# laclouis5/StructureDetector

Hardware: AMD Instinct MI355X
Metric: images/sec (train fwd+bwd) and decode us/img at 512x512 (higher is better)
Workload: dtype f32

## Files before the change

structuredetector_amd/csrc/sd_nn.hip:

```cpp
#include "sd_common.h"
#include "sd_mfma.h"
#include <type_traits>

namespace sd {

constexpr int RED_ROWS_PER_BLOCK = 256;

template <int MODE, typename T = float>
__global__ __launch_bounds__(256) void k_col_reduce(const T* __restrict__ a, const T* __restrict__ b, const T* __restrict__ y,
                                                     const float* __restrict__ mean, const float* __restrict__ invstd,
                                                     const float* __restrict__ gamma, const float* __restrict__ beta, int relu,
                                                     int64_t M, int C, float* __restrict__ partial, int rpb) {
    __shared__ float4 red[2][256];
    const int cols = C >> 2;
    const int lanes = 256 / cols;
    const int col = threadIdx.x % cols, rl = threadIdx.x / cols;
    const int64_t r0 = (int64_t)blockIdx.x * rpb;
    const int64_t r1 = min(r0 + rpb, M);
    float4 s0 = make_float4(0.f, 0.f, 0.f, 0.f), s1 = s0;
    float4 mu = s0, is = s0, ga = s0, be = s0;
    if (MODE == 1 && rl < lanes) {
        mu = reinterpret_cast<const float4*>(mean)[col];
        is = reinterpret_cast<const float4*>(invstd)[col];
        if (relu == 2) { ga = reinterpret_cast<const float4*>(gamma)[col]; be = reinterpret_cast<const float4*>(beta)[col]; }
    }
    if (rl < lanes) {
#pragma unroll 4
        for (int64_t r = r0 + rl; r < r1; r += lanes) {
            const float4 v = ld4(a, r * cols + col);
            if (MODE == 0) {
                s0.x += v.x; s0.y += v.y; s0.z += v.z; s0.w += v.w;
                s1.x += v.x * v.x; s1.y += v.y * v.y; s1.z += v.z * v.z; s1.w += v.w * v.w;
            } else if (MODE == 2) {
                s0.x += v.x; s0.y += v.y; s0.z += v.z; s0.w += v.w;
            } else {
                float4 g = v;
                const float4 xv = ld4(b, r * cols + col);
                if (relu == 1) {
                    const float4 yy = ld4(y, r * cols + col);
                    g.x = yy.x > 0.f ? g.x : 0.f; g.y = yy.y > 0.f ? g.y : 0.f;
                    g.z = yy.z > 0.f ? g.z : 0.f; g.w = yy.w > 0.f ? g.w : 0.f;
                } else if (relu == 2) {
                    g.x = ((xv.x - mu.x) * is.x * ga.x + be.x) > 0.f ? g.x : 0.f; g.y = ((xv.y - mu.y) * is.y * ga.y + be.y) > 0.f ? g.y : 0.f;
                    g.z = ((xv.z - mu.z) * is.z * ga.z + be.z) > 0.f ? g.z : 0.f; g.w = ((xv.w - mu.w) * is.w * ga.w + be.w) > 0.f ? g.w : 0.f;
                } else if (relu == 3) {
                    const uint8_t mb = reinterpret_cast<const uint8_t*>(y)[r * cols + col];
                    g.x = (mb & 1) ? g.x : 0.f; g.y = (mb & 2) ? g.y : 0.f; g.z = (mb & 4) ? g.z : 0.f; g.w = (mb & 8) ? g.w : 0.f;
                }
                s0.x += g.x; s0.y += g.y; s0.z += g.z; s0.w += g.w;
                s1.x += g.x * ((xv.x - mu.x) * is.x); s1.y += g.y * ((xv.y - mu.y) * is.y);
                s1.z += g.z * ((xv.z - mu.z) * is.z); s1.w += g.w * ((xv.w - mu.w) * is.w);
            }
        }
    }
    red[0][threadIdx.x] = s0;
    red[1][threadIdx.x] = s1;
    __syncthreads();
    if (rl == 0) {
        for (int l = 1; l < lanes; ++l) {
            const float4 u = red[0][l * cols + col], w = red[1][l * cols + col];
            s0.x += u.x; s0.y += u.y; s0.z += u.z; s0.w += u.w;
            s1.x += w.x; s1.y += w.y; s1.z += w.z; s1.w += w.w;
        }
        float* dst = partial + (int64_t)blockIdx.x * 2 * C;
        reinterpret_cast<float4*>(dst)[col] = s0;
        reinterpret_cast<float4*>(dst + C)[col] = s1;
    }
}

__global__ __launch_bounds__(256) void k_rows_fold(const float* __restrict__ in, int rows, int W, int slab, float* __restrict__ out) {
    __shared__ float4 red[256];
    const int cols = W >> 2, lanes = 256 / cols;
    const int col = threadIdx.x % cols, rl = threadIdx.x / cols;
    const int r0 = blockIdx.x * slab, r1 = min(r0 + slab, rows);
    float4 s = make_float4(0.f, 0.f, 0.f, 0.f);
    if (rl < lanes) {
#pragma unroll 4
        for (int r = r0 + rl; r < r1; r += lanes) {
            const float4 v = reinterpret_cast<const float4*>(in + (int64_t)r * W)[col];
            s.x += v.x; s.y += v.y; s.z += v.z; s.w += v.w;
        }
    }
    red[threadIdx.x] = s;
    __syncthreads();
    if (rl == 0) {
        for (int l = 1; l < lanes; ++l) { const float4 u = red[l * cols + col]; s.x += u.x; s.y += u.y; s.z += u.z; s.w += u.w; }
        reinterpret_cast<float4*>(out + (int64_t)blockIdx.x * W)[col] = s;
    }
}

__device__ __forceinline__ bool col_pair_sums(const float* __restrict__ partial, int nblocks, int C, double (&r0)[4][4], double (&r1)[4][4],
                                              double& s0, double& s1) {
    const int lc = threadIdx.x & 3, lr = threadIdx.x >> 2;
    const int c = blockIdx.x * 4 + lc;
    s0 = 0.0; s1 = 0.0;
    if (c < C) {
        double t0[8] = {0, 0, 0, 0, 0, 0, 0, 0}, t1[8] = {0, 0, 0, 0, 0, 0, 0, 0};
        for (int b = lr; b < nblocks; b += 64 * 8) {
            float v0[8], v1[8];
#pragma unroll
            for (int u = 0; u < 8; ++u) {
                const int row = b + 64 * u;
                const int64_t o = (int64_t)(row < nblocks ? row : 0) * 2 * C + c;
                v0[u] = partial[o];
                v1[u] = partial[o + C];
            }
#pragma unroll
            for (int u = 0; u < 8; ++u) {
                const bool ok = b + 64 * u < nblocks;
                t0[u] += ok ? (double)v0[u] : 0.0; t1[u] += ok ? (double)v1[u] : 0.0;
            }
        }
        s0 = ((t0[0] + t0[1]) + (t0[2] + t0[3])) + ((t0[4] + t0[5]) + (t0[6] + t0[7]));
        s1 = ((t1[0] + t1[1]) + (t1[2] + t1[3])) + ((t1[4] + t1[5]) + (t1[6] + t1[7]));
    }
#pragma unroll
    for (int o = 4; o < 64; o <<= 1) { s0 += __shfl_xor(s0, o); s1 += __shfl_xor(s1, o); }
// ... 26 lines not shown
    __shared__ double r0[4][4], r1[4][4];
    double s0, s1;
    if (!col_pair_sums(partial, nblocks, C, r0, r1, s0, s1)) return;
    const int c = blockIdx.x * 4 + (threadIdx.x & 3);
    if (FIN == 0) {
        bn_stats_tail(s0, s1, M, eps, momentum, c, out0, out1, run_mean, run_var);
    } else if (FIN == 1) {
        out0[c] = (accumulate ? out0[c] : 0.f) + (float)s1;
        out1[c] = (accumulate ? out1[c] : 0.f) + (float)s0;
        aux0[c] = (float)(s0 / M);
        aux1[c] = (float)(s1 / M);
    } else {
        out0[c] = (accumulate ? out0[c] : 0.f) + (float)s0;
    }
}

template <int FIN>
__global__ __launch_bounds__(256) void k_col_sums(const float* __restrict__ partial, int nblocks, int C, double M, float* __restrict__ dgamma,
                                                   float* __restrict__ dbeta, int accumulate, double* __restrict__ sums) {
    __shared__ double r0[4][4], r1[4][4];
    double s0, s1;
    if (!col_pair_sums(partial, nblocks, C, r0, r1, s0, s1)) return;
    const int c = blockIdx.x * 4 + (threadIdx.x & 3);
    sums[c] = s0;
    sums[C + c] = s1;
    if (c == 0) sums[2 * C] = M;
    if (FIN == 1) {
        dgamma[c] = (accumulate ? dgamma[c] : 0.f) + (float)s1;
        dbeta[c] = (accumulate ? dbeta[c] : 0.f) + (float)s0;
    }
}

__global__ __launch_bounds__(256) void k_bn_stats_from_sums(const double* __restrict__ sums, int C, float eps, float momentum,
                                                             float* __restrict__ mean, float* __restrict__ invstd,
                                                             float* __restrict__ run_mean, float* __restrict__ run_var) {
    const int c = blockIdx.x * 256 + threadIdx.x;
    if (c >= C) return;
    bn_stats_tail(sums[c], sums[C + c], sums[2 * C], eps, momentum, c, mean, invstd, run_mean, run_var);
}

__global__ __launch_bounds__(256) void k_bn_bwd_means_from_sums(const double* __restrict__ sums, int C, float* __restrict__ means) {
    const int c = blockIdx.x * 256 + threadIdx.x;
    if (c >= C) return;
    const double M = sums[2 * C];
    means[c] = (float)(sums[c] / M);
    means[C + c] = (float)(sums[C + c] / M);
}

template <typename T>
__global__ __launch_bounds__(256) void k_bn_apply(const T* __restrict__ x, T* __restrict__ y, int64_t n4, int C,
                                                   const float* __restrict__ mean, const float* __restrict__ invstd,
                                                   const float* __restrict__ gamma, const float* __restrict__ beta,
                                                   const T* __restrict__ res, int relu, uint8_t* __restrict__ mask) {
    const int64_t stride = (int64_t)gridDim.x * 256;
    const int cols = C >> 2;
    const bool fixed = stride % cols == 0;
    const int col0 = (int)(((int64_t)blockIdx.x * 256 + threadIdx.x) % cols);
    float4 mu = reinterpret_cast<const float4*>(mean)[col0], is = reinterpret_cast<const float4*>(invstd)[col0];
    float4 g = reinterpret_cast<const float4*>(gamma)[col0], b = reinterpret_cast<const float4*>(beta)[col0];
    for (int64_t i = (int64_t)blockIdx.x * 256 + threadIdx.x; i < n4; i += stride) {
        const float4 v = ld4(x, i);
        if (!fixed) {
            const int col = (int)(i % cols);
            mu = reinterpret_cast<const float4*>(mean)[col]; is = reinterpret_cast<const float4*>(invstd)[col];
            g = reinterpret_cast<const float4*>(gamma)[col]; b = reinterpret_cast<const float4*>(beta)[col];
        }
        float4 o;
        o.x = (v.x - mu.x) * is.x * g.x + b.x; o.y = (v.y - mu.y) * is.y * g.y + b.y;
        o.z = (v.z - mu.z) * is.z * g.z + b.z; o.w = (v.w - mu.w) * is.w * g.w + b.w;
        if (res) {
            const float4 r = ld4(res, i);
            o.x += r.x; o.y += r.y; o.z += r.z; o.w += r.w;
        }
        if (mask) mask[i] = (uint8_t)((o.x > 0.f ? 1 : 0) | (o.y > 0.f ? 2 : 0) | (o.z > 0.f ? 4 : 0) | (o.w > 0.f ? 8 : 0));
        if (relu) { o.x = fmaxf(o.x, 0.f); o.y = fmaxf(o.y, 0.f); o.z = fmaxf(o.z, 0.f); o.w = fmaxf(o.w, 0.f); }
        st4(y, i, o);
    }
}

__global__ __launch_bounds__(256) void k_bn_fold(const float* gamma, const float* beta, const float* rm, const float* rv, float eps,
                                                  int C, float* scale, float* shift) {
    const int c = blockIdx.x * 256 + threadIdx.x;
    if (c >= C) return;
    const float s = gamma[c] / sqrtf(rv[c] + eps);
    scale[c] = s;
    shift[c] = beta[c] - rm[c] * s;
}

template <typename T>
__global__ __launch_bounds__(256) void k_bn_bwd_apply(const T* __restrict__ dy, const T* __restrict__ x, const T* __restrict__ y,
                                                       int relu, int64_t n4, int C, const float* __restrict__ mean,
                                                       const float* __restrict__ invstd, const float* __restrict__ gamma,
                                                       const float* __restrict__ beta, const float* __restrict__ mg,
                                                       const float* __restrict__ mgx, T* __restrict__ dx, T* __restrict__ g_out) {
    const int64_t stride = (int64_t)gridDim.x * 256;
    const int cols = C >> 2;
    const bool fixed = stride % cols == 0;
    const int col0 = (int)(((int64_t)blockIdx.x * 256 + threadIdx.x) % cols);
    float4 mu = reinterpret_cast<const float4*>(mean)[col0], is = reinterpret_cast<const float4*>(invstd)[col0];
    float4 ga = reinterpret_cast<const float4*>(gamma)[col0];
    float4 be = relu == 2 ? reinterpret_cast<const float4*>(beta)[col0] : make_float4(0.f, 0.f, 0.f, 0.f);
    float4 a = reinterpret_cast<const float4*>(mg)[col0], b = reinterpret_cast<const float4*>(mgx)[col0];
    for (int64_t i = (int64_t)blockIdx.x * 256 + threadIdx.x; i < n4; i += stride) {
        float4 g = ld4(dy, i);
        const float4 xv = ld4(x, i);
        if (!fixed) {
            const int col = (int)(i % cols);
            mu = reinterpret_cast<const float4*>(mean)[col]; is = reinterpret_cast<const float4*>(invstd)[col];
            ga = reinterpret_cast<const float4*>(gamma)[col];
            if (relu == 2) be = reinterpret_cast<const float4*>(beta)[col];
            a = reinterpret_cast<const float4*>(mg)[col]; b = reinterpret_cast<const float4*>(mgx)[col];
        }
        if (relu == 1) {
            const float4 yy = ld4(y, i);
            g.x = yy.x > 0.f ? g.x : 0.f; g.y = yy.y > 0.f ? g.y : 0.f; g.z = yy.z > 0.f ? g.z : 0.f; g.w = yy.w > 0.f ? g.w : 0.f;
        } else if (relu == 3) {
            const uint8_t mb = reinterpret_cast<const uint8_t*>(y)[i];
            g.x = (mb & 1) ? g.x : 0.f; g.y = (mb & 2) ? g.y : 0.f; g.z = (mb & 4) ? g.z : 0.f; g.w = (mb & 8) ? g.w : 0.f;
        } else if (relu == 2) {
            g.x = ((xv.x - mu.x) * is.x * ga.x + be.x) > 0.f ? g.x : 0.f; g.y = ((xv.y - mu.y) * is.y * ga.y + be.y) > 0.f ? g.y : 0.f;
            g.z = ((xv.z - mu.z) * is.z * ga.z + be.z) > 0.f ? g.z : 0.f; g.w = ((xv.w - mu.w) * is.w * ga.w + be.w) > 0.f ? g.w : 0.f;
        }
        float4 o;
        o.x = ga.x * is.x * (g.x - a.x - (xv.x - mu.x) * is.x * b.x);
        o.y = ga.y * is.y * (g.y - a.y - (xv.y - mu.y) * is.y * b.y);
        o.z = ga.z * is.z * (g.z - a.z - (xv.z - mu.z) * is.z * b.z);
        o.w = ga.w * is.w * (g.w - a.w - (xv.w - mu.w) * is.w * b.w);
        st4(dx, i, o);
        if (g_out) st4(g_out, i, g);
    }
}

__global__ __launch_bounds__(256) void k_maxpool_fwd(const float* __restrict__ x, float* __restrict__ y, uint8_t* __restrict__ idx, int B,
                                                      int Hi, int Wi, int Ho, int Wo, int C) {
    const int cols = C >> 2;
    const int64_t n4 = (int64_t)B * Ho * Wo * cols;
    const int64_t i = (int64_t)blockIdx.x * 256 + threadIdx.x;
    if (i >= n4) return;
    const int col = (int)(i % cols);
    int64_t t = i / cols;
    const int ox = (int)(t % Wo); t /= Wo;
    const int oy = (int)(t % Ho);
    const int b = (int)(t / Ho);
    float4 m = make_float4(-INFINITY, -INFINITY, -INFINITY, -INFINITY);
    uchar4 w = make_uchar4(0, 0, 0, 0);
#pragma unroll
    for (int r = 0; r < 3; ++r) {
#pragma unroll
        for (int s = 0; s < 3; ++s) {
            const int iy = oy * 2 - 1 + r, ix = ox * 2 - 1 + s;
            if (iy < 0 || iy >= Hi || ix < 0 || ix >= Wi) continue;
            const float4 v = reinterpret_cast<const float4*>(x + (((int64_t)b * Hi + iy) * Wi + ix) * C)[col];
            const uint8_t tap = (uint8_t)(r * 3 + s);
            if (v.x > m.x) { m.x = v.x; w.x = tap; }
            if (v.y > m.y) { m.y = v.y; w.y = tap; }
            if (v.z > m.z) { m.z = v.z; w.z = tap; }
// ... 50 lines not shown
    int64_t t = i / cols;
    const int ox = (int)(t % Wo); t /= Wo;
    const int oy = (int)(t % Ho);
    const int b = (int)(t / Ho);
    const float4 mu = reinterpret_cast<const float4*>(mean)[col], is = reinterpret_cast<const float4*>(invstd)[col];
    const float4 ga = reinterpret_cast<const float4*>(gamma)[col], be = reinterpret_cast<const float4*>(beta)[col];
    float4 m = make_float4(-INFINITY, -INFINITY, -INFINITY, -INFINITY);
    uchar4 w = make_uchar4(0, 0, 0, 0);
#pragma unroll
    for (int r = 0; r < 3; ++r) {
#pragma unroll
        for (int s = 0; s < 3; ++s) {
            const int iy = oy * 2 - 1 + r, ix = ox * 2 - 1 + s;
            if (iy < 0 || iy >= Hi || ix < 0 || ix >= Wi) continue;
            const float4 xv = ld4(x, (((int64_t)b * Hi + iy) * Wi + ix) * cols + col);
            float4 v;
            v.x = fmaxf((xv.x - mu.x) * is.x * ga.x + be.x, 0.f); v.y = fmaxf((xv.y - mu.y) * is.y * ga.y + be.y, 0.f);
            v.z = fmaxf((xv.z - mu.z) * is.z * ga.z + be.z, 0.f); v.w = fmaxf((xv.w - mu.w) * is.w * ga.w + be.w, 0.f);
            const uint8_t tap = (uint8_t)(r * 3 + s);
            if (v.x > m.x) { m.x = v.x; w.x = tap; }
            if (v.y > m.y) { m.y = v.y; w.y = tap; }
            if (v.z > m.z) { m.z = v.z; w.z = tap; }
            if (v.w > m.w) { m.w = v.w; w.w = tap; }
        }
    }
    st4(y, i, m);
    reinterpret_cast<uchar4*>(idx)[i] = w;
}

template <int VEC> struct PoolVec { float v[VEC]; };
__device__ __forceinline__ PoolVec<4> pool_ld(const float* p, int64_t e) {
    const float4 r = *reinterpret_cast<const float4*>(p + e);
    return PoolVec<4>{{r.x, r.y, r.z, r.w}};
}
__device__ __forceinline__ PoolVec<8> pool_ld(const uint16_t* p, int64_t e) {
    const uint4 r = *reinterpret_cast<const uint4*>(p + e);
    return PoolVec<8>{{bf16_to_f32((uint16_t)(r.x & 0xffff)), bf16_to_f32((uint16_t)(r.x >> 16)), bf16_to_f32((uint16_t)(r.y & 0xffff)), bf16_to_f32((uint16_t)(r.y >> 16)),
                       bf16_to_f32((uint16_t)(r.z & 0xffff)), bf16_to_f32((uint16_t)(r.z >> 16)), bf16_to_f32((uint16_t)(r.w & 0xffff)), bf16_to_f32((uint16_t)(r.w >> 16))}};
}
__device__ __forceinline__ void pool_st(float* p, int64_t e, const PoolVec<4>& m) { *reinterpret_cast<float4*>(p + e) = make_float4(m.v[0], m.v[1], m.v[2], m.v[3]); }
__device__ __forceinline__ void pool_st(uint16_t* p, int64_t e, const PoolVec<8>& m) {
    uint4 r;
    r.x = (uint32_t)f32_to_bf16(m.v[0]) | ((uint32_t)f32_to_bf16(m.v[1]) << 16); r.y = (uint32_t)f32_to_bf16(m.v[2]) | ((uint32_t)f32_to_bf16(m.v[3]) << 16);
    r.z = (uint32_t)f32_to_bf16(m.v[4]) | ((uint32_t)f32_to_bf16(m.v[5]) << 16); r.w = (uint32_t)f32_to_bf16(m.v[6]) | ((uint32_t)f32_to_bf16(m.v[7]) << 16);
    *reinterpret_cast<uint4*>(p + e) = r;
}
template <typename XT, typename PT, int VEC>
__global__ __launch_bounds__(256) void k_bn_relu_maxpool_fwd_pair(const XT* __restrict__ x, const float* __restrict__ mean,
                                                                   const float* __restrict__ invstd, const float* __restrict__ gamma,
                                                                   const float* __restrict__ beta, PT* __restrict__ y,
                                                                   uint8_t* __restrict__ idx, int B, int Hi, int Wi, int Ho, int Wo, int C) {
    const int cols = C / VEC, Wp = Wo >> 1;
    const int64_t n = (int64_t)B * Ho * Wp * cols;
    const int64_t i = (int64_t)blockIdx.x * 256 + threadIdx.x;
    if (i >= n) return;
    const int col = (int)(i % cols);
    int64_t t = i / cols;
    const int oxp = (int)(t % Wp); t /= Wp;
    const int oy = (int)(t % Ho);
    const int b = (int)(t / Ho);
    float mu[VEC], is[VEC], ga[VEC], be[VEC];
#pragma unroll
    for (int k = 0; k < VEC; ++k) { mu[k] = mean[col * VEC + k]; is[k] = invstd[col * VEC + k]; ga[k] = gamma[col * VEC + k]; be[k] = beta[col * VEC + k]; }
    PoolVec<VEC> m0, m1;
    uint8_t w0[VEC], w1[VEC];
#pragma unroll
    for (int k = 0; k < VEC; ++k) { m0.v[k] = m1.v[k] = -INFINITY; w0[k] = w1[k] = 0; }
#pragma unroll
    for (int r = 0; r < 3; ++r) {
        const int iy = oy * 2 - 1 + r;
        if (iy < 0 || iy >= Hi) continue;
#pragma unroll
        for (int c = 0; c < 5; ++c) {
            const int ix = oxp * 4 - 1 + c;
            if (ix < 0 || ix >= Wi) continue;
            const PoolVec<VEC> xv = pool_ld(x, (((int64_t)b * Hi + iy) * Wi + ix) * C + col * VEC);
#pragma unroll
            for (int k = 0; k < VEC; ++k) {
                const float v = fmaxf((xv.v[k] - mu[k]) * is[k] * ga[k] + be[k], 0.f);
                if (c <= 2 && v > m0.v[k]) { m0.v[k] = v; w0[k] = (uint8_t)(r * 3 + c); }
                if (c >= 2 && v > m1.v[k]) { m1.v[k] = v; w1[k] = (uint8_t)(r * 3 + c - 2); }
            }
        }
    }
    const int64_t o = (((int64_t)b * Ho + oy) * Wo + 2 * oxp) * C + col * VEC;
    pool_st(y, o, m0); pool_st(y, o + C, m1);
    uint32_t p0[VEC / 4], p1[VEC / 4];
#pragma unroll
    for (int k = 0; k < VEC / 4; ++k) {
        p0[k] = w0[4 * k] | ((uint32_t)w0[4 * k + 1] << 8) | ((uint32_t)w0[4 * k + 2] << 16) | ((uint32_t)w0[4 * k + 3] << 24);
        p1[k] = w1[4 * k] | ((uint32_t)w1[4 * k + 1] << 8) | ((uint32_t)w1[4 * k + 2] << 16) | ((uint32_t)w1[4 * k + 3] << 24);
    }
#pragma unroll
    for (int k = 0; k < VEC / 4; ++k) { reinterpret_cast<uint32_t*>(idx + o)[k] = p0[k]; reinterpret_cast<uint32_t*>(idx + o + C)[k] = p1[k]; }
}

__device__ __forceinline__ float4 pool_relu_grad(const float* __restrict__ dpool, const uint8_t* __restrict__ idx, int b, int iy, int ix,
                                                 int col, int cols, int Ho, int Wo, const float4 xv, const float4 mu, const float4 is,
                                                 const float4 ga, const float4 be) {
    float4 acc = make_float4(0.f, 0.f, 0.f, 0.f);
    for (int oy = (iy + 1) / 2 - ((iy + 1) % 2 == 0 ? 1 : 0); oy <= (iy + 1) / 2; ++oy) {
        if (oy < 0 || oy >= Ho) continue;
        const int r = iy - (oy * 2 - 1);
        if (r < 0 || r > 2) continue;
        for (int ox = (ix + 1) / 2 - ((ix + 1) % 2 == 0 ? 1 : 0); ox <= (ix + 1) / 2; ++ox) {
            if (ox < 0 || ox >= Wo) continue;
            const int s = ix - (ox * 2 - 1);
// ... 6 lines not shown
            if (w.y == tap) acc.y += g.y;
            if (w.z == tap) acc.z += g.z;
            if (w.w == tap) acc.w += g.w;
        }
    }
    acc.x = ((xv.x - mu.x) * is.x * ga.x + be.x) > 0.f ? acc.x : 0.f; acc.y = ((xv.y - mu.y) * is.y * ga.y + be.y) > 0.f ? acc.y : 0.f;
    acc.z = ((xv.z - mu.z) * is.z * ga.z + be.z) > 0.f ? acc.z : 0.f; acc.w = ((xv.w - mu.w) * is.w * ga.w + be.w) > 0.f ? acc.w : 0.f;
    return acc;
}

template <typename PT>
__device__ __forceinline__ void pool_relu_grad_quad(const PT* __restrict__ dpool, const uint8_t* __restrict__ idx, int b, int k, int j,
                                                    int col, int cols, int Ho, int Wo, const float4* xv, const float4 mu, const float4 is,
                                                    const float4 ga, const float4 be, float4* g) {
    const bool hy = k + 1 < Ho, hx = j + 1 < Wo;
    const int64_t o00 = (((int64_t)b * Ho + k) * Wo + j) * cols + col;
    const int64_t o01 = hx ? o00 + cols : o00, o10 = hy ? o00 + (int64_t)Wo * cols : o00, o11 = (hx && hy) ? o00 + (int64_t)(Wo + 1) * cols : o00;
    const uchar4 w00 = reinterpret_cast<const uchar4*>(idx)[o00], w01 = reinterpret_cast<const uchar4*>(idx)[o01];
    const uchar4 w10 = reinterpret_cast<const uchar4*>(idx)[o10], w11 = reinterpret_cast<const uchar4*>(idx)[o11];
    const float4 d00 = ld4(dpool, o00);
    float4 d01 = ld4(dpool, o01), d10 = ld4(dpool, o10);
    float4 d11 = ld4(dpool, o11);
    const float4 z = make_float4(0.f, 0.f, 0.f, 0.f);
    if (!hx) d01 = z;
    if (!hy) d10 = z;
    if (!(hx && hy)) d11 = z;
#define SD_PICK(W, D, TAP) make_float4((W).x == (TAP) ? (D).x : 0.f, (W).y == (TAP) ? (D).y : 0.f, (W).z == (TAP) ? (D).z : 0.f, (W).w == (TAP) ? (D).w : 0.f)
#define SD_ADD4(A, B) { (A).x += (B).x; (A).y += (B).y; (A).z += (B).z; (A).w += (B).w; }
    g[0] = SD_PICK(w00, d00, 4);
    g[1] = SD_PICK(w00, d00, 5); { const float4 t = SD_PICK(w01, d01, 3); SD_ADD4(g[1], t) }
    g[2] = SD_PICK(w00, d00, 7); { const float4 t = SD_PICK(w10, d10, 1); SD_ADD4(g[2], t) }
    g[3] = SD_PICK(w00, d00, 8);
    { const float4 t = SD_PICK(w01, d01, 6); SD_ADD4(g[3], t) }
    { const float4 t = SD_PICK(w10, d10, 2); SD_ADD4(g[3], t) }
    { const float4 t = SD_PICK(w11, d11, 0); SD_ADD4(g[3], t) }
#undef SD_PICK
#pragma unroll
    for (int q = 0; q < 4; ++q) {
        g[q].x = ((xv[q].x - mu.x) * is.x * ga.x + be.x) > 0.f ? g[q].x : 0.f; g[q].y = ((xv[q].y - mu.y) * is.y * ga.y + be.y) > 0.f ? g[q].y : 0.f;
        g[q].z = ((xv[q].z - mu.z) * is.z * ga.z + be.z) > 0.f ? g[q].z : 0.f; g[q].w = ((xv[q].w - mu.w) * is.w * ga.w + be.w) > 0.f ? g[q].w : 0.f;
    }
}

template <typename XT, typename PT>
__global__ __launch_bounds__(256) void k_pool_bn_bwd_reduce_quad(const PT* __restrict__ dpool, const uint8_t* __restrict__ idx,
                                                                  const XT* __restrict__ x, const float* __restrict__ mean,
                                                                  const float* __restrict__ invstd, const float* __restrict__ gamma,
                                                                  const float* __restrict__ beta, int Hi, int Wi, int Ho, int Wo, int64_t MQ,
                                                                  int C, float* __restrict__ partial) {
    __shared__ float4 red[2][256];
    const int cols = C >> 2, lanes = 256 / cols;
    const int col = threadIdx.x % cols, rl = threadIdx.x / cols;
    constexpr int QPB = RED_ROWS_PER_BLOCK / 4;
    const int64_t q0 = (int64_t)blockIdx.x * QPB, q1 = min(q0 + QPB, MQ);
    const int Hq = Hi >> 1, Wq = Wi >> 1;
    float4 s0 = make_float4(0.f, 0.f, 0.f, 0.f), s1 = s0;
    if (rl < lanes) {
        const float4 mu = reinterpret_cast<const float4*>(mean)[col], is = reinterpret_cast<const float4*>(invstd)[col];
        const float4 ga = reinterpret_cast<const float4*>(gamma)[col], be = reinterpret_cast<const float4*>(beta)[col];
        for (int64_t q = q0 + rl; q < q1; q += lanes) {
            const int j = (int)(q % Wq);
            const int64_t t = q / Wq;
            const int k = (int)(t % Hq), b = (int)(t / Hq);
            const int64_t p00 = (((int64_t)b * Hi + 2 * k) * Wi + 2 * j) * cols + col;
            float4 xv[4], g[4];
            xv[0] = ld4(x, p00); xv[1] = ld4(x, p00 + cols);
            xv[2] = ld4(x, p00 + (int64_t)Wi * cols); xv[3] = ld4(x, p00 + (int64_t)(Wi + 1) * cols);
            pool_relu_grad_quad(dpool, idx, b, k, j, col, cols, Ho, Wo, xv, mu, is, ga, be, g);
#pragma unroll
            for (int u = 0; u < 4; ++u) {
                s0.x += g[u].x; s0.y += g[u].y; s0.z += g[u].z; s0.w += g[u].w;
                s1.x += g[u].x * ((xv[u].x - mu.x) * is.x); s1.y += g[u].y * ((xv[u].y - mu.y) * is.y);
                s1.z += g[u].z * ((xv[u].z - mu.z) * is.z); s1.w += g[u].w * ((xv[u].w - mu.w) * is.w);
            }
        }
    }
    red[0][threadIdx.x] = s0;
    red[1][threadIdx.x] = s1;
    __syncthreads();
    if (rl == 0) {
        for (int l = 1; l < lanes; ++l) {
            const float4 u = red[0][l * cols + col], w = red[1][l * cols + col];
            s0.x += u.x; s0.y += u.y; s0.z += u.z; s0.w += u.w;
            s1.x += w.x; s1.y += w.y; s1.z += w.z; s1.w += w.w;
        }
        float* dst = partial + (int64_t)blockIdx.x * 2 * C;
        reinterpret_cast<float4*>(dst)[col] = s0;
        reinterpret_cast<float4*>(dst + C)[col] = s1;
    }
}

template <typename XT, typename PT, typename DT = float>
__global__ __launch_bounds__(256) void k_pool_bn_bwd_apply_quad(const PT* __restrict__ dpool, const uint8_t* __restrict__ idx,
                                                                 const XT* __restrict__ x, const float* __restrict__ mean,
                                                                 const float* __restrict__ invstd, const float* __restrict__ gamma,
                                                                 const float* __restrict__ beta, const float* __restrict__ mg,
                                                                 const float* __restrict__ mgx, int Hi, int Wi, int Ho, int Wo, int64_t nq4,
                                                                 int C, DT* __restrict__ dx) {
    const int64_t i = (int64_t)blockIdx.x * 256 + threadIdx.x;
    if (i >= nq4) return;
    const int cols = C >> 2;
    const int col = (int)(i % cols);
    const int64_t q = i / cols;
    const int Hq = Hi >> 1, Wq = Wi >> 1;
    const int j = (int)(q % Wq);
    const int64_t t = q / Wq;
    const int k = (int)(t % Hq), b = (int)(t / Hq);
    const float4 mu = reinterpret_cast<const float4*>(mean)[col], is = reinterpret_cast<const float4*>(invstd)[col];
    const float4 ga = reinterpret_cast<const float4*>(gamma)[col], be = reinterpret_cast<const float4*>(beta)[col];
    const float4 a = reinterpret_cast<const float4*>(mg)[col], bb = reinterpret_cast<const float4*>(mgx)[col];
    const int64_t p00 = (((int64_t)b * Hi + 2 * k) * Wi + 2 * j) * cols + col;
    const int64_t off[4] = {p00, p00 + cols, p00 + (int64_t)Wi * cols, p00 + (int64_t)(Wi + 1) * cols};
    float4 xv[4], g[4];
#pragma unroll
    for (int u = 0; u < 4; ++u) xv[u] = ld4(x, off[u]);
    pool_relu_grad_quad(dpool, idx, b, k, j, col, cols, Ho, Wo, xv, mu, is, ga, be, g);
#pragma unroll
    for (int u = 0; u < 4; ++u) {
        float4 o;
        o.x = ga.x * is.x * (g[u].x - a.x - (xv[u].x - mu.x) * is.x * bb.x);
        o.y = ga.y * is.y * (g[u].y - a.y - (xv[u].y - mu.y) * is.y * bb.y);
        o.z = ga.z * is.z * (g[u].z - a.z - (xv[u].z - mu.z) * is.z * bb.z);
        o.w = ga.w * is.w * (g[u].w - a.w - (xv[u].w - mu.w) * is.w * bb.w);
        st4(dx, off[u], o);
    }
}
#undef SD_ADD4

__global__ __launch_bounds__(256) void k_pool_bn_bwd_reduce(const float* __restrict__ dpool, const uint8_t* __restrict__ idx,
                                                             const float* __restrict__ x, const float* __restrict__ mean,
                                                             const float* __restrict__ invstd, const float* __restrict__ gamma,
                                                             const float* __restrict__ beta, int Hi, int Wi, int Ho, int Wo, int64_t M,
                                                             int C, float* __restrict__ partial) {
    __shared__ float4 red[2][256];
    const int cols = C >> 2, lanes = 256 / cols;
    const int col = threadIdx.x % cols, rl = threadIdx.x / cols;
    const int64_t r0 = (int64_t)blockIdx.x * RED_ROWS_PER_BLOCK, r1 = min(r0 + RED_ROWS_PER_BLOCK, M);
    float4 s0 = make_float4(0.f, 0.f, 0.f, 0.f), s1 = s0;
    if (rl < lanes) {
        const float4 mu = reinterpret_cast<const float4*>(mean)[col], is = reinterpret_cast<const float4*>(invstd)[col];
        const float4 ga = reinterpret_cast<const float4*>(gamma)[col], be = reinterpret_cast<const float4*>(beta)[col];
        for (int64_t r = r0 + rl; r < r1; r += lanes) {
            const int ix = (int)(r % Wi);
            const int64_t t = r / Wi;
            const int iy = (int)(t % Hi), b = (int)(t / Hi);
            const float4 xv = reinterpret_cast<const float4*>(x + r * C)[col];
            const float4 g = pool_relu_grad(dpool, idx, b, iy, ix, col, cols, Ho, Wo, xv, mu, is, ga, be);
            s0.x += g.x; s0.y += g.y; s0.z += g.z; s0.w += g.w;
            s1.x += g.x * ((xv.x - mu.x) * is.x); s1.y += g.y * ((xv.y - mu.y) * is.y);
            s1.z += g.z * ((xv.z - mu.z) * is.z); s1.w += g.w * ((xv.w - mu.w) * is.w);
        }
    }
// ... 753 lines not shown
        for (int st = 0; st < 8; ++st) {
#pragma unroll
            for (int mi = 0; mi < 2; ++mi) {
                const int r = mi * 32 + fr;
                const head_bf16x8 a = *reinterpret_cast<const head_bf16x8*>(reinterpret_cast<const char*>(T) + r * 256 + (((2 * st + fh) ^ (r & 15)) << 4));
                acc[mi] = __builtin_amdgcn_mfma_f32_32x32x16_bf16(a, bh[st], acc[mi], 0, 0, 0);
                if (SPLIT) accl[mi] = __builtin_amdgcn_mfma_f32_32x32x16_bf16(a, bl[st], accl[mi], 0, 0, 0);
            }
        }
        asm volatile("s_waitcnt lgkmcnt(0)" ::: "memory");
#pragma unroll
        for (int mi = 0; mi < 2; ++mi) {
#pragma unroll
            for (int g = 0; g < 4; ++g) {
                float4 o;
                float* op = &o.x;
#pragma unroll
                for (int k = 0; k < 4; ++k) {
                    const float hi = acc[mi][4 * g + k];
                    const float lo = SPLIT ? accl[mi][4 * g + k] : __shfl_down(hi, 16);
                    op[k] = hi + lo + bv;
                }
                const int64_t m = m0 + mi * 32 + 8 * g + 4 * fh;
                if (fr < Co && (SPLIT || fr < 16) && m < M) {
                    const int64_t b = m / HW, pix = m - b * HW;
                    *reinterpret_cast<float4*>(y + (b * Co + fr) * HW + pix) = o;
                }
            }
        }
    }
}

struct F8 { float4 a, b; };
__device__ __forceinline__ F8 ld8(const uint16_t* p, int64_t i) {
    typedef unsigned sd_u32x4_nt __attribute__((ext_vector_type(4)));
    const sd_u32x4_nt r_ = __builtin_nontemporal_load(reinterpret_cast<const sd_u32x4_nt*>(p) + i);
    const uint4 r = make_uint4(r_[0], r_[1], r_[2], r_[3]);
    F8 v;
    v.a = make_float4(bf16_to_f32((uint16_t)(r.x & 0xffff)), bf16_to_f32((uint16_t)(r.x >> 16)), bf16_to_f32((uint16_t)(r.y & 0xffff)), bf16_to_f32((uint16_t)(r.y >> 16)));
    v.b = make_float4(bf16_to_f32((uint16_t)(r.z & 0xffff)), bf16_to_f32((uint16_t)(r.z >> 16)), bf16_to_f32((uint16_t)(r.w & 0xffff)), bf16_to_f32((uint16_t)(r.w >> 16)));
    return v;
}
__device__ __forceinline__ void st8(uint16_t* p, int64_t i, const F8& v) {
    uint4 r;
    r.x = (uint32_t)f32_to_bf16(v.a.x) | ((uint32_t)f32_to_bf16(v.a.y) << 16); r.y = (uint32_t)f32_to_bf16(v.a.z) | ((uint32_t)f32_to_bf16(v.a.w) << 16);
    r.z = (uint32_t)f32_to_bf16(v.b.x) | ((uint32_t)f32_to_bf16(v.b.y) << 16); r.w = (uint32_t)f32_to_bf16(v.b.z) | ((uint32_t)f32_to_bf16(v.b.w) << 16);
    reinterpret_cast<uint4*>(p)[i] = r;
}

__global__ __launch_bounds__(256) void k_bn_apply_bf16x8(const uint16_t* __restrict__ x, uint16_t* __restrict__ y, int64_t n8, int C,
                                                          const float* __restrict__ mean, const float* __restrict__ invstd,
                                                          const float* __restrict__ gamma, const float* __restrict__ beta,
                                                          const uint16_t* __restrict__ res, int relu, uint8_t* __restrict__ mask) {
    const int64_t stride = (int64_t)gridDim.x * 256;
    const int cols = C >> 3;
    const bool fixed = stride % cols == 0;
    const int col0 = (int)(((int64_t)blockIdx.x * 256 + threadIdx.x) % cols);
    float4 mu[2], is[2], g[2], b[2];
#pragma unroll
    for (int h = 0; h < 2; ++h) {
        mu[h] = reinterpret_cast<const float4*>(mean)[2 * col0 + h]; is[h] = reinterpret_cast<const float4*>(invstd)[2 * col0 + h];
        g[h] = reinterpret_cast<const float4*>(gamma)[2 * col0 + h]; b[h] = reinterpret_cast<const float4*>(beta)[2 * col0 + h];
    }
    for (int64_t i = (int64_t)blockIdx.x * 256 + threadIdx.x; i < n8; i += stride) {
        const F8 v = ld8(x, i);
        if (!fixed) {
            const int col = (int)(i % cols);
#pragma unroll
            for (int h = 0; h < 2; ++h) {
                mu[h] = reinterpret_cast<const float4*>(mean)[2 * col + h]; is[h] = reinterpret_cast<const float4*>(invstd)[2 * col + h];
                g[h] = reinterpret_cast<const float4*>(gamma)[2 * col + h]; b[h] = reinterpret_cast<const float4*>(beta)[2 * col + h];
            }
        }
        F8 o;
#pragma unroll
        for (int h = 0; h < 2; ++h) {
            const float4 vv = h ? v.b : v.a;
            float4 oo;
            oo.x = (vv.x - mu[h].x) * is[h].x * g[h].x + b[h].x; oo.y = (vv.y - mu[h].y) * is[h].y * g[h].y + b[h].y;
            oo.z = (vv.z - mu[h].z) * is[h].z * g[h].z + b[h].z; oo.w = (vv.w - mu[h].w) * is[h].w * g[h].w + b[h].w;
            if (h) o.b = oo; else o.a = oo;
        }
        if (res) {
            const F8 r = ld8(res, i);
            o.a.x += r.a.x; o.a.y += r.a.y; o.a.z += r.a.z; o.a.w += r.a.w; o.b.x += r.b.x; o.b.y += r.b.y; o.b.z += r.b.z; o.b.w += r.b.w;
        }
        if (mask) {
            const uint8_t m0 = (uint8_t)((o.a.x > 0.f ? 1 : 0) | (o.a.y > 0.f ? 2 : 0) | (o.a.z > 0.f ? 4 : 0) | (o.a.w > 0.f ? 8 : 0));
            const uint8_t m1 = (uint8_t)((o.b.x > 0.f ? 1 : 0) | (o.b.y > 0.f ? 2 : 0) | (o.b.z > 0.f ? 4 : 0) | (o.b.w > 0.f ? 8 : 0));
            reinterpret_cast<uchar2*>(mask)[i] = make_uchar2(m0, m1);
        }
        if (relu) {
            o.a.x = fmaxf(o.a.x, 0.f); o.a.y = fmaxf(o.a.y, 0.f); o.a.z = fmaxf(o.a.z, 0.f); o.a.w = fmaxf(o.a.w, 0.f);
            o.b.x = fmaxf(o.b.x, 0.f); o.b.y = fmaxf(o.b.y, 0.f); o.b.z = fmaxf(o.b.z, 0.f); o.b.w = fmaxf(o.b.w, 0.f);
        }
        st8(y, i, o);
    }
}

__device__ __forceinline__ float4 bn_mask4(float4 g, const float4 xv, const float4 mu, const float4 is, const float4 ga, const float4 be, int relu, uint8_t mb) {
    if (relu == 3) {
        g.x = (mb & 1) ? g.x : 0.f; g.y = (mb & 2) ? g.y : 0.f; g.z = (mb & 4) ? g.z : 0.f; g.w = (mb & 8) ? g.w : 0.f;
    } else if (relu == 2) {
        g.x = ((xv.x - mu.x) * is.x * ga.x + be.x) > 0.f ? g.x : 0.f; g.y = ((xv.y - mu.y) * is.y * ga.y + be.y) > 0.f ? g.y : 0.f;
        g.z = ((xv.z - mu.z) * is.z * ga.z + be.z) > 0.f ? g.z : 0.f; g.w = ((xv.w - mu.w) * is.w * ga.w + be.w) > 0.f ? g.w : 0.f;
    }
    return g;
}

__global__ __launch_bounds__(256) void k_bn_bwd_apply_bf16x8(const uint16_t* __restrict__ dy, const uint16_t* __restrict__ x, const uint8_t* __restrict__ maskb,
                                                              int relu, int64_t n8, int C, const float* __restrict__ mean,
                                                              const float* __restrict__ invstd, const float* __restrict__ gamma,
                                                              const float* __restrict__ beta, const float* __restrict__ mg,
                                                              const float* __restrict__ mgx, uint16_t* __restrict__ dx, uint16_t* __restrict__ g_out) {
    const int64_t stride = (int64_t)gridDim.x * 256;
    const int cols = C >> 3;
    const bool fixed = stride % cols == 0;
    const int col0 = (int)(((int64_t)blockIdx.x * 256 + threadIdx.x) % cols);
    float4 mu[2], is[2], ga[2], be[2], a[2], b[2];
    auto params = [&](int col) {
#pragma unroll
        for (int h = 0; h < 2; ++h) {
            mu[h] = reinterpret_cast<const float4*>(mean)[2 * col + h]; is[h] = reinterpret_cast<const float4*>(invstd)[2 * col + h];
            ga[h] = reinterpret_cast<const float4*>(gamma)[2 * col + h];
            be[h] = relu == 2 ? reinterpret_cast<const float4*>(beta)[2 * col + h] : make_float4(0.f, 0.f, 0.f, 0.f);
            a[h] = reinterpret_cast<const float4*>(mg)[2 * col + h]; b[h] = reinterpret_cast<const float4*>(mgx)[2 * col + h];
        }
    };
    params(col0);
    for (int64_t i = (int64_t)blockIdx.x * 256 + threadIdx.x; i < n8; i += stride) {
        const F8 gy = ld8(dy, i), xv = ld8(x, i);
        if (!fixed) params((int)(i % cols));
        uchar2 mb = make_uchar2(0, 0);
        if (relu == 3) mb = reinterpret_cast<const uchar2*>(maskb)[i];
        F8 o, gm;
#pragma unroll
        for (int h = 0; h < 2; ++h) {
            const float4 xx = h ? xv.b : xv.a;
            const float4 g = bn_mask4(h ? gy.b : gy.a, xx, mu[h], is[h], ga[h], be[h], relu, h ? mb.y : mb.x);
            float4 oo;
            oo.x = ga[h].x * is[h].x * (g.x - a[h].x - (xx.x - mu[h].x) * is[h].x * b[h].x);
            oo.y = ga[h].y * is[h].y * (g.y - a[h].y - (xx.y - mu[h].y) * is[h].y * b[h].y);
            oo.z = ga[h].z * is[h].z * (g.z - a[h].z - (xx.z - mu[h].z) * is[h].z * b[h].z);
            oo.w = ga[h].w * is[h].w * (g.w - a[h].w - (xx.w - mu[h].w) * is[h].w * b[h].w);
            if (h) { o.b = oo; gm.b = g; } else { o.a = oo; gm.a = g; }
        }
        st8(dx, i, o);
        if (g_out) st8(g_out, i, gm);
    }
}

__global__ __launch_bounds__(256) void k_col_reduce_bwd_bf16x8(const uint16_t* __restrict__ a, const uint16_t* __restrict__ b, const uint8_t* __restrict__ maskb,
                                                                const float* __restrict__ mean, const float* __restrict__ invstd,
                                                                const float* __restrict__ gamma, const float* __restrict__ beta, int relu,
                                                                int64_t M, int C, float* __restrict__ partial, int rpb) {
    __shared__ float4 red[4][256];
    const int cols = C >> 3;
    const int lanes = 256 / cols;
    const int col = threadIdx.x % cols, rl = threadIdx.x / cols;
    const int64_t r0 = (int64_t)blockIdx.x * rpb, r1 = min(r0 + rpb, M);
    float4 s0[2], s1[2], mu[2], is[2], ga[2], be[2];
#pragma unroll
    for (int h = 0; h < 2; ++h) {
        s0[h] = s1[h] = ga[h] = be[h] = make_float4(0.f, 0.f, 0.f, 0.f);
        mu[h] = reinterpret_cast<const float4*>(mean)[2 * col + h]; is[h] = reinterpret_cast<const float4*>(invstd)[2 * col + h];
        if (relu == 2) { ga[h] = reinterpret_cast<const float4*>(gamma)[2 * col + h]; be[h] = reinterpret_cast<const float4*>(beta)[2 * col + h]; }
    }
    if (rl < lanes) {
#pragma unroll 2
        for (int64_t r = r0 + rl; r < r1; r += lanes) {
            const F8 gy = ld8(a, r * cols + col), xv = ld8(b, r * cols + col);
            uchar2 mb = make_uchar2(0, 0);
            if (relu == 3) mb = reinterpret_cast<const uchar2*>(maskb)[r * cols + col];
#pragma unroll
            for (int h = 0; h < 2; ++h) {
                const float4 xx = h ? xv.b : xv.a;
                const float4 g = bn_mask4(h ? gy.b : gy.a, xx, mu[h], is[h], ga[h], be[h], relu, h ? mb.y : mb.x);
                s0[h].x += g.x; s0[h].y += g.y; s0[h].z += g.z; s0[h].w += g.w;
                s1[h].x += g.x * ((xx.x - mu[h].x) * is[h].x); s1[h].y += g.y * ((xx.y - mu[h].y) * is[h].y);
                s1[h].z += g.z * ((xx.z - mu[h].z) * is[h].z); s1[h].w += g.w * ((xx.w - mu[h].w) * is[h].w);
            }
        }
    }
    red[0][threadIdx.x] = s0[0]; red[1][threadIdx.x] = s0[1]; red[2][threadIdx.x] = s1[0]; red[3][threadIdx.x] = s1[1];
    __syncthreads();
    if (rl == 0) {
        for (int l = 1; l < lanes; ++l) {
#pragma unroll
            for (int h = 0; h < 2; ++h) {
                const float4 u = red[h][l * cols + col], w = red[2 + h][l * cols + col];
                s0[h].x += u.x; s0[h].y += u.y; s0[h].z += u.z; s0[h].w += u.w;
                s1[h].x += w.x; s1[h].y += w.y; s1[h].z += w.z; s1[h].w += w.w;
            }
        }
        float* dst = partial + (int64_t)blockIdx.x * 2 * C;
#pragma unroll
        for (int h = 0; h < 2; ++h) {
            reinterpret_cast<float4*>(dst)[2 * col + h] = s0[h];
            reinterpret_cast<float4*>(dst + C)[2 * col + h] = s1[h];
        }
    }
}

__global__ __launch_bounds__(256) void k_bn_frozen_bwd_f32x4(const float* __restrict__ dy, const float* __restrict__ y, const float* __restrict__ scale,
                                                              int64_t n4, int C, float* __restrict__ dx, float* __restrict__ g_out) {
    const int64_t stride = (int64_t)gridDim.x * 256;
    const int64_t i0 = (int64_t)blockIdx.x * 256 + threadIdx.x;
    const int c0 = 4 * (int)(i0 % (C >> 2));
    const float s0 = scale[c0], s1 = scale[c0 + 1], s2 = scale[c0 + 2], s3 = scale[c0 + 3];
    for (int64_t i = i0; i < n4; i += stride) {
        float4 g = ld4(dy, i);
        if (y) {
            const float4 yy = ld4(y, i);
            g.x = yy.x > 0.f ? g.x : 0.f; g.y = yy.y > 0.f ? g.y : 0.f; g.z = yy.z > 0.f ? g.z : 0.f; g.w = yy.w > 0.f ? g.w : 0.f;
        }
        st4(dx, i, make_float4(g.x * s0, g.y * s1, g.z * s2, g.w * s3));
        if (g_out) st4(g_out, i, g);
    }
}

__device__ __forceinline__ uint32_t frozen_mask2(uint32_t d, uint32_t y) {
    return (bf16_to_f32((uint16_t)(y & 0xffffu)) > 0.f ? (d & 0xffffu) : 0u) | (bf16_to_f32((uint16_t)(y >> 16)) > 0.f ? (d & 0xffff0000u) : 0u);
}
__device__ __forceinline__ uint32_t frozen_scale2(uint32_t g, float s0, float s1) {
    return (uint32_t)f32_to_bf16(bf16_to_f32((uint16_t)(g & 0xffffu)) * s0) | ((uint32_t)f32_to_bf16(bf16_to_f32((uint16_t)(g >> 16)) * s1) << 16);
}

__global__ __launch_bounds__(256) void k_bn_frozen_bwd_bf16x8(const uint16_t* __restrict__ dy, const uint16_t* __restrict__ y, const float* __restrict__ scale,
                                                               int64_t n8, int C, uint16_t* __restrict__ dx, uint16_t* __restrict__ g_out) {
    typedef unsigned sd_u32x4_nt __attribute__((ext_vector_type(4)));
    const int64_t stride = (int64_t)gridDim.x * 256;
    const int64_t i0 = (int64_t)blockIdx.x * 256 + threadIdx.x;
    const int c0 = 8 * (int)(i0 % (C >> 3));
    float s[8];
#pragma unroll
    for (int j = 0; j < 8; ++j) s[j] = scale[c0 + j];
    for (int64_t i = i0; i < n8; i += stride) {
        const sd_u32x4_nt d = __builtin_nontemporal_load(reinterpret_cast<const sd_u32x4_nt*>(dy) + i);
        uint4 g = make_uint4(d[0], d[1], d[2], d[3]);
        if (y) {
            const sd_u32x4_nt m = __builtin_nontemporal_load(reinterpret_cast<const sd_u32x4_nt*>(y) + i);
            g = make_uint4(frozen_mask2(g.x, m[0]), frozen_mask2(g.y, m[1]), frozen_mask2(g.z, m[2]), frozen_mask2(g.w, m[3]));
        }
        reinterpret_cast<uint4*>(dx)[i] = make_uint4(frozen_scale2(g.x, s[0], s[1]), frozen_scale2(g.y, s[2], s[3]), frozen_scale2(g.z, s[4], s[5]),
                                                     frozen_scale2(g.w, s[6], s[7]));
        if (g_out) reinterpret_cast<uint4*>(g_out)[i] = g;
    }
}
// ... 948 lines not shown
```

Measured before the change: 875.8.

## Remap BN and pooling block order across XCDs to reuse recently written data in cache

Adds a pass_chunk helper that permutes which row chunk each block processes. Forward BN/reduction kernels visit chunks newest-first within each XCD's contiguous range, and backward apply kernels retrace via xcd_remap. The aim is for consecutive passes to hit data still resident in the per-XCD L2 or infinity cache instead of DRAM. Grid-stride loops become chunk loops, and a compile-time ablation macro plus a KEPT flag turn the remap off for some kernels. This adds index arithmetic and changes the partial-sum write order.

```diff
diff --git a/structuredetector_amd/csrc/sd_nn.hip b/structuredetector_amd/csrc/sd_nn.hip
--- a/structuredetector_amd/csrc/sd_nn.hip
+++ b/structuredetector_amd/csrc/sd_nn.hip
@@ -3,6 +3,20 @@
 #include <type_traits>
 
 namespace sd {
+
+#ifndef SD_PASS_ORDER_ABL
+#define SD_PASS_ORDER_ABL 0
+#endif
+enum PassOrder { PASS_NEWEST_FIRST, PASS_RETRACE };
+template <PassOrder ORDER, bool KEPT = true>
+__device__ __forceinline__ int pass_chunk(int t, int n) {
+    if (SD_PASS_ORDER_ABL == 1 || (!KEPT && SD_PASS_ORDER_ABL != 3)) return t;
+    if (SD_PASS_ORDER_ABL == 2) return ORDER == PASS_NEWEST_FIRST ? n - 1 - t : t;
+    if (ORDER == PASS_RETRACE) return xcd_remap(t, n);
+    const int q = n >> 3, r = n & 7, xcd = t & 7;
+    const int first = xcd < r ? xcd * (q + 1) : r * (q + 1) + (xcd - r) * q, count = q + (xcd < r ? 1 : 0);
+    return first + count - 1 - (t >> 3);
+}
 
 constexpr int RED_ROWS_PER_BLOCK = 256;
 
@@ -15,7 +29,8 @@
     const int cols = C >> 2;
     const int lanes = 256 / cols;
     const int col = threadIdx.x % cols, rl = threadIdx.x / cols;
-    const int64_t r0 = (int64_t)blockIdx.x * rpb;
+    const int rb = pass_chunk<PASS_NEWEST_FIRST>(blockIdx.x, gridDim.x);
+    const int64_t r0 = (int64_t)rb * rpb;
     const int64_t r1 = min(r0 + rpb, M);
     float4 s0 = make_float4(0.f, 0.f, 0.f, 0.f), s1 = s0;
     float4 mu = s0, is = s0, ga = s0, be = s0;
@@ -62,7 +77,7 @@
             s0.x += u.x; s0.y += u.y; s0.z += u.z; s0.w += u.w;
             s1.x += w.x; s1.y += w.y; s1.z += w.z; s1.w += w.w;
         }
-        float* dst = partial + (int64_t)blockIdx.x * 2 * C;
+        float* dst = partial + (int64_t)rb * 2 * C;
         reinterpret_cast<float4*>(dst)[col] = s0;
         reinterpret_cast<float4*>(dst + C)[col] = s1;
     }
@@ -195,13 +210,15 @@
                                                    const float* __restrict__ mean, const float* __restrict__ invstd,
                                                    const float* __restrict__ gamma, const float* __restrict__ beta,
                                                    const T* __restrict__ res, int relu, uint8_t* __restrict__ mask) {
-    const int64_t stride = (int64_t)gridDim.x * 256;
     const int cols = C >> 2;
-    const bool fixed = stride % cols == 0;
-    const int col0 = (int)(((int64_t)blockIdx.x * 256 + threadIdx.x) % cols);
+    const bool fixed = 256 % cols == 0;
+    const int col0 = (int)(threadIdx.x % cols);
     float4 mu = reinterpret_cast<const float4*>(mean)[col0], is = reinterpret_cast<const float4*>(invstd)[col0];
     float4 g = reinterpret_cast<const float4*>(gamma)[col0], b = reinterpret_cast<const float4*>(beta)[col0];
-    for (int64_t i = (int64_t)blockIdx.x * 256 + threadIdx.x; i < n4; i += stride) {
+    const int nchunk = (int)((n4 + 255) >> 8);
+    for (int t = blockIdx.x; t < nchunk; t += gridDim.x) {
+        const int64_t i = (int64_t)pass_chunk<PASS_NEWEST_FIRST>(t, nchunk) * 256 + threadIdx.x;
+        if (i >= n4) continue;
         const float4 v = ld4(x, i);
         if (!fixed) {
             const int col = (int)(i % cols);
@@ -236,15 +253,17 @@
                                                        const float* __restrict__ invstd, const float* __restrict__ gamma,
                                                        const float* __restrict__ beta, const float* __restrict__ mg,
                                                        const float* __restrict__ mgx, T* __restrict__ dx, T* __restrict__ g_out) {
-    const int64_t stride = (int64_t)gridDim.x * 256;
     const int cols = C >> 2;
-    const bool fixed = stride % cols == 0;
-    const int col0 = (int)(((int64_t)blockIdx.x * 256 + threadIdx.x) % cols);
+    const bool fixed = 256 % cols == 0;
+    const int col0 = (int)(threadIdx.x % cols);
     float4 mu = reinterpret_cast<const float4*>(mean)[col0], is = reinterpret_cast<const float4*>(invstd)[col0];
     float4 ga = reinterpret_cast<const float4*>(gamma)[col0];
     float4 be = relu == 2 ? reinterpret_cast<const float4*>(beta)[col0] : make_float4(0.f, 0.f, 0.f, 0.f);
     float4 a = reinterpret_cast<const float4*>(mg)[col0], b = reinterpret_cast<const float4*>(mgx)[col0];
-    for (int64_t i = (int64_t)blockIdx.x * 256 + threadIdx.x; i < n4; i += stride) {
+    const int nchunk = (int)((n4 + 255) >> 8);
+    for (int t = blockIdx.x; t < nchunk; t += gridDim.x) {
+        const int64_t i = (int64_t)pass_chunk<PASS_RETRACE>(t, nchunk) * 256 + threadIdx.x;
+        if (i >= n4) continue;
         float4 g = ld4(dy, i);
         const float4 xv = ld4(x, i);
         if (!fixed) {
@@ -401,7 +420,7 @@
                                                                    uint8_t* __restrict__ idx, int B, int Hi, int Wi, int Ho, int Wo, int C) {
     const int cols = C / VEC, Wp = Wo >> 1;
     const int64_t n = (int64_t)B * Ho * Wp * cols;
-    const int64_t i = (int64_t)blockIdx.x * 256 + threadIdx.x;
+    const int64_t i = (int64_t)pass_chunk<PASS_NEWEST_FIRST>(blockIdx.x, gridDim.x) * 256 + threadIdx.x;
     if (i >= n) return;
     const int col = (int)(i % cols);
     int64_t t = i / cols;
@@ -514,7 +533,8 @@
     const int cols = C >> 2, lanes = 256 / cols;
     const int col = threadIdx.x % cols, rl = threadIdx.x / cols;
     constexpr int QPB = RED_ROWS_PER_BLOCK / 4;
-    const int64_t q0 = (int64_t)blockIdx.x * QPB, q1 = min(q0 + QPB, MQ);
+    const int rb = pass_chunk<PASS_NEWEST_FIRST, false>(blockIdx.x, gridDim.x);
+    const int64_t q0 = (int64_t)rb * QPB, q1 = min(q0 + QPB, MQ);
     const int Hq = Hi >> 1, Wq = Wi >> 1;
     float4 s0 = make_float4(0.f, 0.f, 0.f, 0.f), s1 = s0;
     if (rl < lanes) {
@@ -546,7 +566,7 @@
             s0.x += u.x; s0.y += u.y; s0.z += u.z; s0.w += u.w;
             s1.x += w.x; s1.y += w.y; s1.z += w.z; s1.w += w.w;
         }
-        float* dst = partial + (int64_t)blockIdx.x * 2 * C;
+        float* dst = partial + (int64_t)rb * 2 * C;
         reinterpret_cast<float4*>(dst)[col] = s0;
         reinterpret_cast<float4*>(dst + C)[col] = s1;
     }
@@ -559,7 +579,7 @@
                                                                  const float* __restrict__ beta, const float* __restrict__ mg,
                                                                  const float* __restrict__ mgx, int Hi, int Wi, int Ho, int Wo, int64_t nq4,
                                                                  int C, DT* __restrict__ dx) {
-    const int64_t i = (int64_t)blockIdx.x * 256 + threadIdx.x;
+    const int64_t i = (int64_t)pass_chunk<PASS_RETRACE, false>(blockIdx.x, gridDim.x) * 256 + threadIdx.x;
     if (i >= nq4) return;
     const int cols = C >> 2;
     const int col = (int)(i % cols);
@@ -1419,17 +1439,19 @@
                                                           const float* __restrict__ mean, const float* __restrict__ invstd,
                                                           const float* __restrict__ gamma, const float* __restrict__ beta,
                                                           const uint16_t* __restrict__ res, int relu, uint8_t* __restrict__ mask) {
-    const int64_t stride = (int64_t)gridDim.x * 256;
     const int cols = C >> 3;
-    const bool fixed = stride % cols == 0;
-    const int col0 = (int)(((int64_t)blockIdx.x * 256 + threadIdx.x) % cols);
+    const bool fixed = 256 % cols == 0;
+    const int col0 = (int)(threadIdx.x % cols);
     float4 mu[2], is[2], g[2], b[2];
 #pragma unroll
     for (int h = 0; h < 2; ++h) {
         mu[h] = reinterpret_cast<const float4*>(mean)[2 * col0 + h]; is[h] = reinterpret_cast<const float4*>(invstd)[2 * col0 + h];
         g[h] = reinterpret_cast<const float4*>(gamma)[2 * col0 + h]; b[h] = reinterpret_cast<const float4*>(beta)[2 * col0 + h];
     }
-    for (int64_t i = (int64_t)blockIdx.x * 256 + threadIdx.x; i < n8; i += stride) {
+    const int nchunk = (int)((n8 + 255) >> 8);
+    for (int t = blockIdx.x; t < nchunk; t += gridDim.x) {
+        const int64_t i = (int64_t)pass_chunk<PASS_NEWEST_FIRST>(t, nchunk) * 256 + threadIdx.x;
+        if (i >= n8) continue;
         const F8 v = ld8(x, i);
         if (!fixed) {
             const int col = (int)(i % cols);
@@ -1480,10 +1502,9 @@
                                                               const float* __restrict__ invstd, const float* __restrict__ gamma,
                                                               const float* __restrict__ beta, const float* __restrict__ mg,
                                                               const float* __restrict__ mgx, uint16_t* __restrict__ dx, uint16_t* __restrict__ g_out) {
-    const int64_t stride = (int64_t)gridDim.x * 256;
     const int cols = C >> 3;
-    const bool fixed = stride % cols == 0;
-    const int col0 = (int)(((int64_t)blockIdx.x * 256 + threadIdx.x) % cols);
+    const bool fixed = 256 % cols == 0;
+    const int col0 = (int)(threadIdx.x % cols);
     float4 mu[2], is[2], ga[2], be[2], a[2], b[2];
     auto params = [&](int col) {
 #pragma unroll
@@ -1495,7 +1516,10 @@
         }
     };
     params(col0);
-    for (int64_t i = (int64_t)blockIdx.x * 256 + threadIdx.x; i < n8; i += stride) {
+    const int nchunk = (int)((n8 + 255) >> 8);
+    for (int t = blockIdx.x; t < nchunk; t += gridDim.x) {
+        const int64_t i = (int64_t)pass_chunk<PASS_RETRACE, false>(t, nchunk) * 256 + threadIdx.x;
+        if (i >= n8) continue;
         const F8 gy = ld8(dy, i), xv = ld8(x, i);
         if (!fixed) params((int)(i % cols));
         uchar2 mb = make_uchar2(0, 0);
@@ -1525,7 +1549,8 @@
     const int cols = C >> 3;
     const int lanes = 256 / cols;
     const int col = threadIdx.x % cols, rl = threadIdx.x / cols;
-    const int64_t r0 = (int64_t)blockIdx.x * rpb, r1 = min(r0 + rpb, M);
+    const int rb = pass_chunk<PASS_NEWEST_FIRST, false>(blockIdx.x, gridDim.x);
+    const int64_t r0 = (int64_t)rb * rpb, r1 = min(r0 + rpb, M);
     float4 s0[2], s1[2], mu[2], is[2], ga[2], be[2];
 #pragma unroll
     for (int h = 0; h < 2; ++h) {
@@ -1560,7 +1585,7 @@
                 s1[h].x += w.x; s1[h].y += w.y; s1[h].z += w.z; s1[h].w += w.w;
             }
         }
-        float* dst = partial + (int64_t)blockIdx.x * 2 * C;
+        float* dst = partial + (int64_t)rb * 2 * C;
 #pragma unroll
         for (int h = 0; h < 2; ++h) {
             reinterpret_cast<float4*>(dst)[2 * col + h] = s0[h];
```

New measurement: 879.6 (median of 6 runs). Within noise of the previous version (+0.4%).
